# tiantengfei/Distributed-tensorflow-for-DCGAN

Hardware: AMD Instinct MI355X
Metric: images/sec (whole node), 64x64 DCGAN bs=128/GPU at 1/2/4/8 MI355X (higher is better)
Workload: dtype bf16; 1 GPU; model=DCGAN-64x64x3 (G 5,135,363 / D 4,316,545 params), global_batch=128, per_gpu_batch=128, parallelism=dp1, engine=hip, hip_graph=False, schedule=fused, backend=none, world_size=1

## Files before the change

### csrc/hip/narrow2.hip

```cpp
#include "kernels.h"

#if defined(DCG_F32)
extern "C" int DCG_API(dcg_nconv)(const elem_t*, const elem_t*, const float*, elem_t*, int, int, int, int, int, int,
                                  int, int, int, float, int, const elem_t*, const elem_t*, const float*, const float*,
                                  int, float, float*, hipStream_t) { return -2; }
extern "C" int DCG_API(dcg_nconv_tiles)(int, int, int) { return -1; }
extern "C" int DCG_API(dcg_nwgrad_plan)(int, int, int, int, int*, int*, int*) { return -1; }
extern "C" int DCG_API(dcg_nwgrad)(const elem_t*, int, int, int, int, const elem_t*, int, int, int, int, float*,
                                   hipStream_t) { return -2; }
extern "C" int DCG_API(dcg_narrow_deconv_dact)(const elem_t*, const elem_t*, elem_t*, const elem_t*, int, int, int, int,
                                               int, int, int, int, int, float, float*, hipStream_t) { return -2; }
extern "C" int DCG_API(dcg_narrow_deconv_tiles)(int, int, int) { return -1; }
extern "C" int DCG_API(dcg_wgrad3_taps_per_tile)(int) { return 1; }
extern "C" int DCG_API(dcg_narrow_deconv_bnin)(const elem_t*, const elem_t*, const float*, elem_t*, int, int, int, int,
                                               int, int, int, int, int, float, const float*, const float*, int, float,
                                               elem_t*, hipStream_t) { return -2; }
#else

namespace dcg {

constexpr int NC_TY = 4;
constexpr int NC_TX = 32;
constexpr int NC_WR = 2 * NC_TY + 3;
constexpr int NC_WC = 2 * NC_TX + 3;
constexpr int NC_WP = NC_WC + 1;
constexpr int NC_WPIX = NC_WR * NC_WC;
constexpr int NC_PPT = (NC_WPIX + 255) / 256;
constexpr int NC_KS = 136;
constexpr int NC_CS = 72;
constexpr int NC_SP = NC_TY * NC_TX * 8 / 256;

struct NConvArgs {
  const elem_t* x; const elem_t* w; const float* bias; elem_t* y;
  int H, W, Ho, Wo, pad_y, pad_x, act; float leak;
  int tiles_x, tiles_per_img, ntiles;
  const elem_t* bx; const elem_t* by; const float* mean; const float* rstd; int bact; float bleak;
  float* part;
};

template <int ACT>
__device__ __forceinline__ float nc_act(float v, float leak) {
  if constexpr (ACT == ACT_RELU) return fmaxf(v, 0.f);
  else if constexpr (ACT == ACT_LRELU) return fmaxf(v, leak * v);
  else if constexpr (ACT == ACT_TANH) return tanhf(v);
  else return v;
}

template <int CIN, bool BNB, int ACT>
__global__ __launch_bounds__(256) void nconv_kernel(NConvArgs p) {
  __shared__ __attribute__((aligned(16))) elem_t wt[64 * NC_KS];
  __shared__ __attribute__((aligned(16))) elem_t xs[NC_WR * NC_WP * 4];
  __shared__ float red[4][2][64];
  __shared__ __attribute__((aligned(16))) elem_t ct[NC_TY * NC_TX * NC_CS];
  const int tid = threadIdx.x, lane = tid & 63, wave = __builtin_amdgcn_readfirstlane(tid >> 6);
  const int li = lane & 15, g = lane >> 4;
  int t = blockIdx.x;
  if (t >= p.ntiles) return;

  for (int q = tid; q < 64 * NC_KS / 8; q += 256) reinterpret_cast<u32x4*>(wt)[q] = (u32x4){0u, 0u, 0u, 0u};
  __syncthreads();
  for (int q = tid; q < 25 * CIN * 64; q += 256) {
    const int n = q & 63, kk = q >> 6, tap = kk / CIN, c = kk - tap * CIN;
    wt[n * NC_KS + 4 * tap + c] = p.w[q];
  }
  __syncthreads();
  elem8 wf[4][4];
#pragma unroll
  for (int nb = 0; nb < 4; ++nb)
#pragma unroll
    for (int kb = 0; kb < 4; ++kb)
      wf[nb][kb] = *reinterpret_cast<const elem8*>(wt + (16 * nb + li) * NC_KS + 32 * kb + 8 * g);
  float bias_r[4][4];
#pragma unroll
  for (int nb = 0; nb < 4; ++nb)
#pragma unroll
    for (int e = 0; e < 4; ++e) bias_r[nb][e] = p.bias ? p.bias[16 * nb + 4 * g + e] : 0.f;
  const int c8 = tid & 7;
  float mu[8], rs[8], s1[8], s2[8];
#pragma unroll
  for (int e = 0; e < 8; ++e) {
    mu[e] = BNB ? p.mean[8 * c8 + e] : 0.f;
    rs[e] = BNB ? p.rstd[8 * c8 + e] : 0.f;
    s1[e] = 0.f;
    s2[e] = 0.f;
  }
  const float bslope = p.bact == ACT_LRELU ? p.bleak : 0.f;

  elem_t pv[NC_PPT][CIN];
  auto fetch = [&](int tt) {
    const int b = tt / p.tiles_per_img, rem = tt - b * p.tiles_per_img;
    const int ty = rem / p.tiles_x, tx = rem - ty * p.tiles_x;
    const int iy0 = 2 * ty * NC_TY - p.pad_y, ix0 = 2 * tx * NC_TX - p.pad_x;
#pragma unroll
    for (int i = 0; i < NC_PPT; ++i) {
      const int q = tid + 256 * i;
      const int r = q / NC_WC, c = q - r * NC_WC;
      const int iy = iy0 + r, ix = ix0 + c;
      const bool ok = q < NC_WPIX && (unsigned)iy < (unsigned)p.H && (unsigned)ix < (unsigned)p.W;
      const elem_t* src = p.x + (((size_t)b * p.H + (ok ? iy : 0)) * p.W + (ok ? ix : 0)) * CIN;
#pragma unroll
      for (int cc = 0; cc < CIN; ++cc) pv[i][cc] = ok ? src[cc] : (elem_t)0.f;
    }
  };
  auto commit = [&]() {
#pragma unroll
    for (int i = 0; i < NC_PPT; ++i) {
      const int q = tid + 256 * i;
      if (q < NC_WPIX) {
        const int r = q / NC_WC, c = q - r * NC_WC;
        elem4 v = {(elem_t)0.f, (elem_t)0.f, (elem_t)0.f, (elem_t)0.f};
#pragma unroll
        for (int cc = 0; cc < CIN; ++cc) v[cc] = pv[i][cc];
        *reinterpret_cast<elem4*>(xs + (r * NC_WP + c) * 4) = v;
      }
    }
  };
  fetch(t);
  commit();
  __syncthreads();
  for (; t < p.ntiles; t += gridDim.x) {
    const int tn = t + gridDim.x;
    const int b = t / p.tiles_per_img, rem = t - b * p.tiles_per_img;
    const int ty = rem / p.tiles_x, tx = rem - ty * p.tiles_x;
    f32x4 acc[2][4];
#pragma unroll
    for (int h = 0; h < 2; ++h)
#pragma unroll
      for (int nb = 0; nb < 4; ++nb) acc[h][nb] = (f32x4){0.f, 0.f, 0.f, 0.f};
#pragma unroll
    for (int kb = 0; kb < 4; ++kb) {
      const int t0 = min(8 * kb + 2 * g, 24), t1 = min(8 * kb + 2 * g + 1, 24);
      const int off0 = (t0 / 5) * NC_WP + (t0 % 5), off1 = (t1 / 5) * NC_WP + (t1 % 5);
#pragma unroll
      for (int h = 0; h < 2; ++h) {
        const int base = 2 * wave * NC_WP + 2 * (16 * h + li);
        const elem4 a0 = *reinterpret_cast<const elem4*>(xs + (base + off0) * 4);
        const elem4 a1 = *reinterpret_cast<const elem4*>(xs + (base + off1) * 4);
        const elem8 xf = __builtin_shufflevector(a0, a1, 0, 1, 2, 3, 4, 5, 6, 7);
#pragma unroll
        for (int nb = 0; nb < 4; ++nb) acc[h][nb] = DCG_MFMA_16x16x32(wf[nb][kb], xf, acc[h][nb], 0, 0, 0);
      }
    }
    if (tn < p.ntiles) fetch(tn);
#pragma unroll
    for (int h = 0; h < 2; ++h) {
      const int px = wave * NC_TX + 16 * h + li;
#pragma unroll
      for (int nb = 0; nb < 4; ++nb) {
        elem4 ov;
#pragma unroll
        for (int e = 0; e < 4; ++e) ov[e] = f2bf(nc_act<ACT>(acc[h][nb][e] + bias_r[nb][e], p.leak));
        *reinterpret_cast<elem4*>(ct + px * NC_CS + 16 * nb + 4 * g) = ov;
      }
    }
    __syncthreads();
    size_t o[NC_SP];
    bool ok[NC_SP];
#pragma unroll
    for (int i = 0; i < NC_SP; ++i) {
      const int px = (tid >> 3) + 32 * i;
      const int oy = ty * NC_TY + (px >> 5), ox = tx * NC_TX + (px & 31);
      ok[i] = oy < p.Ho && ox < p.Wo;
      o[i] = ok[i] ? (((size_t)b * p.Ho + oy) * p.Wo + ox) * 64 + 8 * c8 : 0;
    }
    elem8 bxv[NC_SP], byv[NC_SP];
    if constexpr (BNB) {
#pragma unroll
      for (int i = 0; i < NC_SP; ++i) {
        bxv[i] = *reinterpret_cast<const elem8*>(p.bx + o[i]);
        byv[i] = *reinterpret_cast<const elem8*>(p.by + o[i]);
      }
    }
#pragma unroll
    for (int i = 0; i < NC_SP; ++i) {
      const int px = (tid >> 3) + 32 * i;
      const u32x4 v = *reinterpret_cast<const u32x4*>(ct + px * NC_CS + 8 * c8);
      if (ok[i]) {
        *reinterpret_cast<u32x4*>(p.y + o[i]) = v;
        if constexpr (BNB) {
          const elem8 dv = __builtin_bit_cast(elem8, v);
#pragma unroll
          for (int e = 0; e < 8; ++e) {
            const float gv = (float)dv[e] * ((float)byv[i][e] > 0.f ? 1.f : bslope);
            s1[e] += gv;
            s2[e] += gv * ((float)bxv[i][e] - mu[e]) * rs[e];
          }
        }
      }
    }
    if (tn < p.ntiles) {
      commit();
      __syncthreads();
    }
  }
  if constexpr (BNB) {
#pragma unroll
    for (int e = 0; e < 8; ++e) {
      float a = s1[e], c = s2[e];
#pragma unroll
      for (int sh = 8; sh < 64; sh <<= 1) {
        a += __shfl_xor(a, sh, 64);
        c += __shfl_xor(c, sh, 64);
      }
      if (lane < 8) {
        red[wave][0][8 * c8 + e] = a;
        red[wave][1][8 * c8 + e] = c;
      }
    }
    __syncthreads();
    if (tid < 128) {
      const int st = tid >> 6, n = tid & 63;
      p.part[(size_t)blockIdx.x * 128 + tid] = ((red[0][st][n] + red[1][st][n]) + red[2][st][n]) + red[3][st][n];
    }
  }
}

constexpr int NWG_PX = 256;
constexpr int NWG_WIN = 2048;
constexpr int NWG_WPT = NWG_WIN / 256;

struct NWGradArgs {
  const elem_t* x; int H, W;
  const elem_t* d; int Hd, Wd;
  int pl;
  int tyc, np, nks;
  int wrows, wcols;
  int chunks_per_wg, wg_per_img;
  float* part;
};

__device__ __forceinline__ int nwg_swz(int r) {
  return 4 * (((r >> 1) & 1) | (((r >> 3) & 1) << 1));
}

template <int CIN>
__global__ __launch_bounds__(256) void nwgrad_kernel(NWGradArgs p) {
  extern __shared__ __attribute__((aligned(16))) char smem[];
  char* dt = smem;
  char* win = smem + NWG_PX * 128;
  const int tid = threadIdx.x, lane = tid & 63, wave = __builtin_amdgcn_readfirstlane(tid >> 6);
  const int li = lane & 15, g = lane >> 4, q = li >> 2, pp = li & 3;
  const int b = blockIdx.x / p.wg_per_img;
  const int yb = (blockIdx.x - b * p.wg_per_img) * p.chunks_per_wg * p.tyc;
  const int zero_pix = p.wrows * p.wcols;
  if (tid == 0) *reinterpret_cast<elem4*>(win + zero_pix * 8) = (elem4){(elem_t)0.f, (elem_t)0.f, (elem_t)0.f, (elem_t)0.f};

  int pxoff[8][2];
#pragma unroll
  for (int ks = 0; ks < 8; ++ks)
#pragma unroll
    for (int h = 0; h < 2; ++h) {
      const int px = min(32 * ks + 8 * g + 4 * h + q, p.np - 1);
      const int yy = px / p.Wd, xx = px - yy * p.Wd;
      pxoff[ks][h] = 2 * yy * p.wcols + 2 * xx;
    }
  const int mb0 = 2 * wave, nmb = wave < 3 ? 2 : 1;
  int tapoff[2];
  bool tapok[2];
#pragma unroll
  for (int i = 0; i < 2; ++i) {
    const int tap = 4 * (mb0 + i) + pp;
    tapok[i] = tap < 25;
    tapoff[i] = tapok[i] ? (tap / 5) * p.wcols + (tap % 5) : 0;
  }

  u32x4 dv[NWG_PX * 8 / 256];
  elem_t xv[NWG_WPT][CIN];
  int w_off[NWG_WPT], w_row[NWG_WPT];
#pragma unroll
  for (int i = 0; i < NWG_WPT; ++i) {
    const int s_ = tid + 256 * i;
    const int wr = s_ / p.wcols, wc = s_ - wr * p.wcols, ix = wc - p.pl;
    const bool col_ok = s_ < zero_pix && (unsigned)ix < (unsigned)p.W;
    w_row[i] = col_ok ? wr : -(1 << 20);
    w_off[i] = (wr * p.W + ix) * CIN;
  }
  auto fetch = [&](int y0) {
    const elem_t* dsrc = p.d + ((size_t)b * p.Hd + y0) * p.Wd * 64;
    const int lim = min(p.tyc, p.Hd - y0) * p.Wd * 64;
#pragma unroll
    for (int i = 0; i < NWG_PX * 8 / 256; ++i) {
      const int e0 = (tid + 256 * i) * 8;
      dv[i] = e0 < lim ? *reinterpret_cast<const u32x4*>(dsrc + e0) : (u32x4){0u, 0u, 0u, 0u};
    }
    const int iy0 = 2 * y0 - p.pl;
    const long long xbase = ((long long)b * p.H + iy0) * p.W * CIN;
#pragma unroll
    for (int i = 0; i < NWG_WPT; ++i) {
      const bool ok = (unsigned)(iy0 + w_row[i]) < (unsigned)p.H;
#pragma unroll
      for (int cc = 0; cc < CIN; ++cc) xv[i][cc] = ok ? p.x[xbase + w_off[i] + cc] : (elem_t)0.f;
    }
  };
  auto commit = [&]() {
#pragma unroll
    for (int i = 0; i < NWG_PX * 8 / 256; ++i) {
      const int qd = tid + 256 * i, px = qd >> 3, j = qd & 7;
      *reinterpret_cast<u32x4*>(dt + px * 128 + ((j ^ (nwg_swz(px) >> 1)) << 4)) = dv[i];
    }
#pragma unroll
    for (int i = 0; i < NWG_WPT; ++i) {
      const int s = tid + 256 * i;
      if (s < zero_pix) {
        elem4 v = {(elem_t)0.f, (elem_t)0.f, (elem_t)0.f, (elem_t)0.f};
#pragma unroll
        for (int cc = 0; cc < CIN; ++cc) v[cc] = xv[i][cc];
        *reinterpret_cast<elem4*>(win + s * 8) = v;
      }
    }
  };

  f32x4 acc[2][4];
#pragma unroll
  for (int i = 0; i < 2; ++i)
#pragma unroll
    for (int nb = 0; nb < 4; ++nb) acc[i][nb] = (f32x4){0.f, 0.f, 0.f, 0.f};

  const lds_char* dt3 = (const lds_char*)dt;
  const lds_char* win3 = (const lds_char*)win;
  int nch = 0;
  for (int c = 0; c < p.chunks_per_wg; ++c) nch += (yb + c * p.tyc < p.Hd) ? 1 : 0;
  if (nch > 0) {
    fetch(yb);
    commit();
  }
  __syncthreads();
  for (int c = 0; c < nch; ++c) {
    if (c + 1 < nch) fetch(yb + (c + 1) * p.tyc);
#pragma unroll
    for (int ks = 0; ks < 8; ++ks) {
      if (ks >= p.nks) break;
      elem8 bfr[4];
#pragma unroll
      for (int nb = 0; nb < 4; ++nb)
#pragma unroll
        for (int h = 0; h < 2; ++h) {
          const int r = 32 * ks + 8 * g + 4 * h + q;
          const s16x4 v = __builtin_amdgcn_ds_read_tr16_b64_v4i16(
              LDS_PTR(s16x4, dt3 + r * 128 + (((4 * nb + pp) ^ nwg_swz(r)) << 3)));
          const elem4 vb = __builtin_bit_cast(elem4, v);
#pragma unroll
          for (int e = 0; e < 4; ++e) bfr[nb][4 * h + e] = vb[e];
        }
#pragma unroll
      for (int i = 0; i < 2; ++i) {
        if (i < nmb) {
          elem8 af;
#pragma unroll
          for (int h = 0; h < 2; ++h) {
            const int pix = tapok[i] ? pxoff[ks][h] + tapoff[i] : zero_pix;
            const s16x4 v = __builtin_amdgcn_ds_read_tr16_b64_v4i16(LDS_PTR(s16x4, win3 + pix * 8));
            const elem4 va = __builtin_bit_cast(elem4, v);
#pragma unroll
            for (int e = 0; e < 4; ++e) af[4 * h + e] = va[e];
          }
#pragma unroll
          for (int nb = 0; nb < 4; ++nb) acc[i][nb] = DCG_MFMA_16x16x32(af, bfr[nb], acc[i][nb], 0, 0, 0);
        }
      }
    }
    __syncthreads();
    if (c + 1 < nch) {
      commit();
      __syncthreads();
    }
  }
  float* dst = p.part + (size_t)blockIdx.x * 25 * CIN * 64;
#pragma unroll
  for (int i = 0; i < 2; ++i) {
    if (i < nmb) {
      const int tap = 4 * (mb0 + i) + g;
      if (tap < 25) {
#pragma unroll
        for (int nb = 0; nb < 4; ++nb)
#pragma unroll
          for (int e = 0; e < CIN; ++e) dst[(tap * CIN + e) * 64 + 16 * nb + li] = acc[i][nb][e];
      }
    }
  }
}

}

using namespace dcg;

extern "C" int DCG_API(dcg_nconv)(const elem_t* x, const elem_t* w, const float* bias, elem_t* y, int B, int H, int W,
                                  int Cin, int Ho, int Wo, int pad_y, int pad_x, int act, float leak, int grid,
                                  const elem_t* bx, const elem_t* by, const float* mean, const float* rstd, int bact,
                                  float bleak, float* part, hipStream_t s) {
  if (Cin < 1 || Cin > 4 || pad_y < 0 || pad_y > 2 || pad_x < 0 || pad_x > 2) return -2;
  if (Ho != (H + 1) / 2 || Wo != (W + 1) / 2) return -2;
  NConvArgs a{};
  a.x = x; a.w = w; a.bias = bias; a.y = y;
  a.H = H; a.W = W; a.Ho = Ho; a.Wo = Wo; a.pad_y = pad_y; a.pad_x = pad_x; a.act = act; a.leak = leak;
  a.tiles_x = (Wo + NC_TX - 1) / NC_TX;
  a.tiles_per_img = a.tiles_x * ((Ho + NC_TY - 1) / NC_TY);
  a.ntiles = B * a.tiles_per_img;
  if (grid < 1 || grid > a.ntiles) return -2;
  a.bx = bx; a.by = by; a.mean = mean; a.rstd = rstd; a.bact = bact; a.bleak = bleak; a.part = part;
  const bool bnb = bx != nullptr;
  if (bnb && (!by || !mean || !rstd || !part)) return -2;
#define NC_ACT(CI, BB)                                                                              \
  switch (act) {                                                                                    \
    case ACT_RELU: hipLaunchKernelGGL((nconv_kernel<CI, BB, ACT_RELU>), dim3(grid), dim3(256), 0, s, a); break;   \
    case ACT_LRELU: hipLaunchKernelGGL((nconv_kernel<CI, BB, ACT_LRELU>), dim3(grid), dim3(256), 0, s, a); break; \
    case ACT_TANH: hipLaunchKernelGGL((nconv_kernel<CI, BB, ACT_TANH>), dim3(grid), dim3(256), 0, s, a); break;   \
    default: hipLaunchKernelGGL((nconv_kernel<CI, BB, ACT_NONE>), dim3(grid), dim3(256), 0, s, a); break;         \
  }
#define NC_LAUNCH(CI)    \
  if (bnb) {             \
    NC_ACT(CI, true)     \
  } else {               \
    NC_ACT(CI, false)    \
  }
  switch (Cin) {
    case 1: NC_LAUNCH(1) break;
    case 2: NC_LAUNCH(2) break;
    case 3: NC_LAUNCH(3) break;
    default: NC_LAUNCH(4) break;
  }
#undef NC_LAUNCH
#undef NC_ACT
  return (int)hipGetLastError();
}

extern "C" int DCG_API(dcg_nconv_tiles)(int B, int Ho, int Wo) {
  return B * ((Wo + NC_TX - 1) / NC_TX) * ((Ho + NC_TY - 1) / NC_TY);
}

extern "C" int DCG_API(dcg_nwgrad_plan)(int H, int W, int Hd, int Wd, int* tyc, int* wrows, int* wcols) {
  if (Wd < 1 || Wd > NWG_PX || Hd < 1 || W > 2 * Wd + 1 || H > 2 * Hd + 1) return -1;
  const int t = NWG_PX / Wd;
  const int wr = 2 * t + 3, wc = 2 * Wd + 3;
  if (wr * wc > NWG_WIN) return -1;
  *tyc = t; *wrows = wr; *wcols = wc;
  return 0;
}

extern "C" int DCG_API(dcg_nwgrad)(const elem_t* x, int B, int H, int W, int Cin, const elem_t* d, int Hd, int Wd,
                                   int pl, int chunks_per_wg, float* part, hipStream_t s) {
  NWGradArgs a{};
  if (Cin < 1 || Cin > 4 || pl < 0 || pl > 2 || chunks_per_wg < 1) return -2;
  if (DCG_API(dcg_nwgrad_plan)(H, W, Hd, Wd, &a.tyc, &a.wrows, &a.wcols)) return -2;
  a.x = x; a.H = H; a.W = W; a.d = d; a.Hd = Hd; a.Wd = Wd; a.pl = pl;
  a.np = a.tyc * Wd;
  a.nks = (a.np + 31) / 32;
  a.chunks_per_wg = chunks_per_wg;
  const int chunks_per_img = (Hd + a.tyc - 1) / a.tyc;
  a.wg_per_img = (chunks_per_img + chunks_per_wg - 1) / chunks_per_wg;
  a.part = part;
  const size_t shm = (size_t)NWG_PX * 128 + (size_t)(a.wrows * a.wcols + 1) * 8;
  const unsigned grid = (unsigned)(B * a.wg_per_img);
#define NW_LAUNCH(CI)                                                                                       \
  {                                                                                                         \
    static bool attr = false;                                                                               \
    if (!attr) {                                                                                            \
      hipError_t e = hipFuncSetAttribute((const void*)nwgrad_kernel<CI>, hipFuncAttributeMaxDynamicSharedMemorySize, \
                                         (int)(NWG_PX * 128 + (NWG_WIN + 1) * 8));                          \
      if (e != hipSuccess) return (int)e;                                                                   \
      attr = true;                                                                                          \
    }                                                                                                       \
    hipLaunchKernelGGL(nwgrad_kernel<CI>, dim3(grid), dim3(256), shm, s, a);                                \
  }
  switch (Cin) {
    case 1: NW_LAUNCH(1) break;
    case 2: NW_LAUNCH(2) break;
    case 3: NW_LAUNCH(3) break;
    default: NW_LAUNCH(4) break;
  }
#undef NW_LAUNCH
  return (int)hipGetLastError();
}
#endif
```

Before: 133,100 images/sec.

## Restructure narrow conv staging: vector row loads, LDS aliasing, prefetched BN operands

```diff
diff --git a/csrc/hip/narrow2.hip b/csrc/hip/narrow2.hip
--- a/csrc/hip/narrow2.hip
+++ b/csrc/hip/narrow2.hip
@@ -36,7 +36,11 @@
   int tiles_x, tiles_per_img, ntiles;
   const elem_t* bx; const elem_t* by; const float* mean; const float* rstd; int bact; float bleak;
   float* part;
+  unsigned x_bytes;
+  unsigned y_img_bytes;
 };
+
+typedef unsigned int nc_u32x4 __attribute__((ext_vector_type(4), aligned(2)));
 
 template <int ACT>
 __device__ __forceinline__ float nc_act(float v, float leak) {
@@ -46,82 +50,145 @@
   else return v;
 }
 
-template <int CIN, bool BNB, int ACT>
-__global__ __launch_bounds__(256) void nconv_kernel(NConvArgs p) {
-  __shared__ __attribute__((aligned(16))) elem_t wt[64 * NC_KS];
+template <int CIN, bool BNB, int ACT, bool FAST>
+__global__ __launch_bounds__(256, 2) void nconv_kernel(NConvArgs p) {
+  __shared__ __attribute__((aligned(16))) elem_t ct[NC_TY * NC_TX * NC_CS];
   __shared__ __attribute__((aligned(16))) elem_t xs[NC_WR * NC_WP * 4];
   __shared__ float red[4][2][64];
-  __shared__ __attribute__((aligned(16))) elem_t ct[NC_TY * NC_TX * NC_CS];
+  __shared__ __attribute__((aligned(16))) float cst[4][64];
+  static_assert(64 * NC_KS <= NC_TY * NC_TX * NC_CS, "the weight matrix is staged in the C tile's LDS");
+  elem_t* const wt = ct;
   const int tid = threadIdx.x, lane = tid & 63, wave = __builtin_amdgcn_readfirstlane(tid >> 6);
   const int li = lane & 15, g = lane >> 4;
   int t = blockIdx.x;
   if (t >= p.ntiles) return;
-
-  for (int q = tid; q < 64 * NC_KS / 8; q += 256) reinterpret_cast<u32x4*>(wt)[q] = (u32x4){0u, 0u, 0u, 0u};
-  __syncthreads();
-  for (int q = tid; q < 25 * CIN * 64; q += 256) {
-    const int n = q & 63, kk = q >> 6, tap = kk / CIN, c = kk - tap * CIN;
-    wt[n * NC_KS + 4 * tap + c] = p.w[q];
-  }
-  __syncthreads();
-  elem8 wf[4][4];
-#pragma unroll
-  for (int nb = 0; nb < 4; ++nb)
-#pragma unroll
-    for (int kb = 0; kb < 4; ++kb)
-      wf[nb][kb] = *reinterpret_cast<const elem8*>(wt + (16 * nb + li) * NC_KS + 32 * kb + 8 * g);
-  float bias_r[4][4];
-#pragma unroll
-  for (int nb = 0; nb < 4; ++nb)
-#pragma unroll
-    for (int e = 0; e < 4; ++e) bias_r[nb][e] = p.bias ? p.bias[16 * nb + 4 * g + e] : 0.f;
   const int c8 = tid & 7;
-  float mu[8], rs[8], s1[8], s2[8];
-#pragma unroll
-  for (int e = 0; e < 8; ++e) {
-    mu[e] = BNB ? p.mean[8 * c8 + e] : 0.f;
-    rs[e] = BNB ? p.rstd[8 * c8 + e] : 0.f;
-    s1[e] = 0.f;
-    s2[e] = 0.f;
-  }
-  const float bslope = p.bact == ACT_LRELU ? p.bleak : 0.f;
-
-  elem_t pv[NC_PPT][CIN];
+
+  auto out_of = [&](int tt, size_t& img, int& o0, int& nv) {
+    const int b = tt / p.tiles_per_img, rem = tt - b * p.tiles_per_img;
+    const int ty = rem / p.tiles_x, tx = rem - ty * p.tiles_x;
+    const int ox = tx * NC_TX + (tid >> 3), oy0 = ty * NC_TY;
+    nv = ox < p.Wo ? min(NC_TY, p.Ho - oy0) : 0;
+    o0 = (oy0 * p.Wo + ox) * 64 + 8 * c8;
+    img = (size_t)b * p.Ho * p.Wo * 64;
+  };
+  const int orow = p.Wo * 64;
+  auto load_bn = [&](size_t img, int o0, int nv, elem8 (&vx)[NC_SP], elem8 (&vy)[NC_SP]) {
+#pragma unroll
+    for (int i = 0; i < NC_SP; ++i) {
+      const size_t o = i < nv ? img + (o0 + i * orow) : 0;
+      vx[i] = *reinterpret_cast<const elem8*>(p.bx + o);
+      vy[i] = *reinterpret_cast<const elem8*>(p.by + o);
+    }
+  };
+
+  elem_t pv[FAST ? 1 : NC_PPT][CIN];
+  u32x4 pw[FAST ? CIN : 1];
+  const int f_g = p.W >> 3, f_r = tid / max(f_g, 1), f_j = tid - f_r * f_g;
+  const bool f_on = f_r < NC_WR;
+  const __amdgpu_buffer_rsrc_t rx = make_rsrc(p.x, FAST ? p.x_bytes : 0u);
   auto fetch = [&](int tt) {
     const int b = tt / p.tiles_per_img, rem = tt - b * p.tiles_per_img;
     const int ty = rem / p.tiles_x, tx = rem - ty * p.tiles_x;
     const int iy0 = 2 * ty * NC_TY - p.pad_y, ix0 = 2 * tx * NC_TX - p.pad_x;
-#pragma unroll
-    for (int i = 0; i < NC_PPT; ++i) {
-      const int q = tid + 256 * i;
-      const int r = q / NC_WC, c = q - r * NC_WC;
-      const int iy = iy0 + r, ix = ix0 + c;
-      const bool ok = q < NC_WPIX && (unsigned)iy < (unsigned)p.H && (unsigned)ix < (unsigned)p.W;
-      const elem_t* src = p.x + (((size_t)b * p.H + (ok ? iy : 0)) * p.W + (ok ? ix : 0)) * CIN;
-#pragma unroll
-      for (int cc = 0; cc < CIN; ++cc) pv[i][cc] = ok ? src[cc] : (elem_t)0.f;
+    if constexpr (FAST) {
+      const int iy = iy0 + f_r;
+      const bool ok = f_on && (unsigned)iy < (unsigned)p.H;
+      const uint32_t off = (uint32_t)(((b * p.H + iy) * p.W + 8 * f_j) * CIN) * 2u;
+#pragma unroll
+      for (int cc = 0; cc < CIN; ++cc) pw[cc] = buf_load16(rx, oob_unless(ok, off + 16u * cc));
+    } else {
+#pragma unroll
+      for (int i = 0; i < NC_PPT; ++i) {
+        const int q = tid + 256 * i;
+        const int r = q / NC_WC, c = q - r * NC_WC;
+        const int iy = iy0 + r, ix = ix0 + c;
+        const bool ok = q < NC_WPIX && (unsigned)iy < (unsigned)p.H && (unsigned)ix < (unsigned)p.W;
+        const elem_t* src = p.x + (((size_t)b * p.H + (ok ? iy : 0)) * p.W + (ok ? ix : 0)) * CIN;
+#pragma unroll
+        for (int cc = 0; cc < CIN; ++cc) pv[i][cc] = ok ? src[cc] : (elem_t)0.f;
+      }
     }
   };
   auto commit = [&]() {
-#pragma unroll
-    for (int i = 0; i < NC_PPT; ++i) {
-      const int q = tid + 256 * i;
-      if (q < NC_WPIX) {
-        const int r = q / NC_WC, c = q - r * NC_WC;
-        elem4 v = {(elem_t)0.f, (elem_t)0.f, (elem_t)0.f, (elem_t)0.f};
-#pragma unroll
-        for (int cc = 0; cc < CIN; ++cc) v[cc] = pv[i][cc];
-        *reinterpret_cast<elem4*>(xs + (r * NC_WP + c) * 4) = v;
+    if constexpr (FAST) {
+      if (f_on) {
+        elem_t ev[8 * CIN];
+#pragma unroll
+        for (int cc = 0; cc < CIN; ++cc) {
+          const elem8 v = __builtin_bit_cast(elem8, pw[cc]);
+#pragma unroll
+          for (int k = 0; k < 8; ++k) ev[8 * cc + k] = v[k];
+        }
+#pragma unroll
+        for (int j = 0; j < 8; ++j) {
+          elem4 v = {(elem_t)0.f, (elem_t)0.f, (elem_t)0.f, (elem_t)0.f};
+#pragma unroll
+          for (int cc = 0; cc < CIN; ++cc) v[cc] = ev[j * CIN + cc];
+          *reinterpret_cast<elem4*>(xs + (f_r * NC_WP + p.pad_x + 8 * f_j + j) * 4) = v;
+        }
+      }
+    } else {
+#pragma unroll
+      for (int i = 0; i < NC_PPT; ++i) {
+        const int q = tid + 256 * i;
+        if (q < NC_WPIX) {
+          const int r = q / NC_WC, c = q - r * NC_WC;
+          elem4 v = {(elem_t)0.f, (elem_t)0.f, (elem_t)0.f, (elem_t)0.f};
+#pragma unroll
+          for (int cc = 0; cc < CIN; ++cc) v[cc] = pv[i][cc];
+          *reinterpret_cast<elem4*>(xs + (r * NC_WP + c) * 4) = v;
+        }
       }
     }
   };
+
+  size_t img;
+  int o0, nv;
+  out_of(t, img, o0, nv);
   fetch(t);
+  elem8 bxv[NC_SP], byv[NC_SP];
+  if constexpr (BNB) load_bn(img, o0, nv, bxv, byv);
+  const int wtap = tid >> 3, wn = tid & 7;
+  u32x4 wv[CIN];
+#pragma unroll
+  for (int cc = 0; cc < CIN; ++cc) {
+    const int row = min(wtap * CIN + cc, 25 * CIN - 1);
+    wv[cc] = *reinterpret_cast<const nc_u32x4*>(p.w + row * 64 + 8 * wn);
+  }
+  const float* cp = tid < 64 ? p.bias : !BNB ? nullptr : tid < 128 ? p.mean : tid < 192 ? p.rstd : nullptr;
+  const float cv = cp ? cp[tid & 63] : 0.f;
+  if constexpr (FAST) {
+    for (int q = tid; q < NC_WR * NC_WP * 4 / 8; q += 256) reinterpret_cast<u32x4*>(xs)[q] = (u32x4){0u, 0u, 0u, 0u};
+    __syncthreads();
+  }
+  cst[tid >> 6][tid & 63] = cv;
+#pragma unroll
+  for (int j = 0; j < 8; ++j) {
+    elem4 v = {(elem_t)0.f, (elem_t)0.f, (elem_t)0.f, (elem_t)0.f};
+#pragma unroll
+    for (int cc = 0; cc < CIN; ++cc) v[cc] = wtap < 25 ? __builtin_bit_cast(elem8, wv[cc])[j] : (elem_t)0.f;
+    *reinterpret_cast<elem4*>(wt + (8 * wn + j) * NC_KS + 4 * wtap) = v;
+  }
+  __syncthreads();
+  elem8 wf[4][4];
+#pragma unroll
+  for (int nb = 0; nb < 4; ++nb)
+#pragma unroll
+    for (int kb = 0; kb < 4; ++kb)
+      wf[nb][kb] = *reinterpret_cast<const elem8*>(wt + (16 * nb + li) * NC_KS + 32 * kb + 8 * g);
+  float s1[8], s2[8];
+#pragma unroll
+  for (int e = 0; e < 8; ++e) {
+    s1[e] = 0.f;
+    s2[e] = 0.f;
+  }
+  const float bslope = p.bact == ACT_LRELU ? p.bleak : 0.f;
   commit();
   __syncthreads();
-  for (; t < p.ntiles; t += gridDim.x) {
+  for (;;) {
     const int tn = t + gridDim.x;
-    const int b = t / p.tiles_per_img, rem = t - b * p.tiles_per_img;
-    const int ty = rem / p.tiles_x, tx = rem - ty * p.tiles_x;
+    const bool more = tn < p.ntiles;
     f32x4 acc[2][4];
 #pragma unroll
     for (int h = 0; h < 2; ++h)
@@ -141,42 +208,47 @@
         for (int nb = 0; nb < 4; ++nb) acc[h][nb] = DCG_MFMA_16x16x32(wf[nb][kb], xf, acc[h][nb], 0, 0, 0);
       }
     }
-    if (tn < p.ntiles) fetch(tn);
+    size_t imgn = 0;
+    int o0n = 0, nvn = 0;
+    elem8 bxn[NC_SP], byn[NC_SP];
+    if (more) {
+      out_of(tn, imgn, o0n, nvn);
+      fetch(tn);
+      if constexpr (BNB) load_bn(imgn, o0n, nvn, bxn, byn);
+    }
 #pragma unroll
     for (int h = 0; h < 2; ++h) {
       const int px = wave * NC_TX + 16 * h + li;
 #pragma unroll
       for (int nb = 0; nb < 4; ++nb) {
+        const f32x4 bs = *reinterpret_cast<const f32x4*>(&cst[0][16 * nb + 4 * g]);
         elem4 ov;
 #pragma unroll
-        for (int e = 0; e < 4; ++e) ov[e] = f2bf(nc_act<ACT>(acc[h][nb][e] + bias_r[nb][e], p.leak));
+        for (int e = 0; e < 4; ++e) ov[e] = f2bf(nc_act<ACT>(acc[h][nb][e] + bs[e], p.leak));
         *reinterpret_cast<elem4*>(ct + px * NC_CS + 16 * nb + 4 * g) = ov;
       }
     }
     __syncthreads();
-    size_t o[NC_SP];
-    bool ok[NC_SP];
-#pragma unroll
-    for (int i = 0; i < NC_SP; ++i) {
-      const int px = (tid >> 3) + 32 * i;
-      const int oy = ty * NC_TY + (px >> 5), ox = tx * NC_TX + (px & 31);
-      ok[i] = oy < p.Ho && ox < p.Wo;
-      o[i] = ok[i] ? (((size_t)b * p.Ho + oy) * p.Wo + ox) * 64 + 8 * c8 : 0;
-    }
-    elem8 bxv[NC_SP], byv[NC_SP];
+    const __amdgpu_buffer_rsrc_t ry = make_rsrc(p.y + img, p.y_img_bytes);
+    float mu[8], rs[8];
     if constexpr (BNB) {
 #pragma unroll
-      for (int i = 0; i < NC_SP; ++i) {
-        bxv[i] = *reinterpret_cast<const elem8*>(p.bx + o[i]);
-        byv[i] = *reinterpret_cast<const elem8*>(p.by + o[i]);
+      for (int h = 0; h < 2; ++h) {
+        const f32x4 m4 = *reinterpret_cast<const f32x4*>(&cst[1][8 * c8 + 4 * h]);
+        const f32x4 r4 = *reinterpret_cast<const f32x4*>(&cst[2][8 * c8 + 4 * h]);
+#pragma unroll
+        for (int e = 0; e < 4; ++e) {
+          mu[4 * h + e] = m4[e];
+          rs[4 * h + e] = r4[e];
+        }
       }
     }
 #pragma unroll
     for (int i = 0; i < NC_SP; ++i) {
       const int px = (tid >> 3) + 32 * i;
       const u32x4 v = *reinterpret_cast<const u32x4*>(ct + px * NC_CS + 8 * c8);
-      if (ok[i]) {
-        *reinterpret_cast<u32x4*>(p.y + o[i]) = v;
+      __builtin_amdgcn_raw_buffer_store_b128(v, ry, oob_unless(i < nv, (uint32_t)(o0 + i * orow) * 2u), 0, 0);
+      if (i < nv) {
         if constexpr (BNB) {
           const elem8 dv = __builtin_bit_cast(elem8, v);
 #pragma unroll
@@ -188,9 +260,19 @@
         }
       }
     }
-    if (tn < p.ntiles) {
-      commit();
-      __syncthreads();
+    if (!more) break;
+    commit();
+    __syncthreads();
+    t = tn;
+    img = imgn;
+    o0 = o0n;
+    nv = nvn;
+    if constexpr (BNB) {
+#pragma unroll
+      for (int i = 0; i < NC_SP; ++i) {
+        bxv[i] = bxn[i];
+        byv[i] = byn[i];
+      }
     }
   }
   if constexpr (BNB) {
@@ -400,18 +482,28 @@
   a.bx = bx; a.by = by; a.mean = mean; a.rstd = rstd; a.bact = bact; a.bleak = bleak; a.part = part;
   const bool bnb = bx != nullptr;
   if (bnb && (!by || !mean || !rstd || !part)) return -2;
-#define NC_ACT(CI, BB)                                                                              \
+  const size_t x_bytes = (size_t)B * H * W * Cin * sizeof(elem_t);
+  const bool fast = a.tiles_x == 1 && W % 8 == 0 && ((uintptr_t)x & 15) == 0 && x_bytes < OOB;
+  a.x_bytes = fast ? (unsigned)x_bytes : 0u;
+  const size_t y_img_bytes = (size_t)Ho * Wo * 64 * sizeof(elem_t);
+  if (y_img_bytes >= OOB) return -2;
+  a.y_img_bytes = (unsigned)y_img_bytes;
+#define NC_ACT(CI, BB, FF)                                                                          \
   switch (act) {                                                                                    \
-    case ACT_RELU: hipLaunchKernelGGL((nconv_kernel<CI, BB, ACT_RELU>), dim3(grid), dim3(256), 0, s, a); break;   \
-    case ACT_LRELU: hipLaunchKernelGGL((nconv_kernel<CI, BB, ACT_LRELU>), dim3(grid), dim3(256), 0, s, a); break; \
-    case ACT_TANH: hipLaunchKernelGGL((nconv_kernel<CI, BB, ACT_TANH>), dim3(grid), dim3(256), 0, s, a); break;   \
-    default: hipLaunchKernelGGL((nconv_kernel<CI, BB, ACT_NONE>), dim3(grid), dim3(256), 0, s, a); break;         \
-  }
-#define NC_LAUNCH(CI)    \
-  if (bnb) {             \
-    NC_ACT(CI, true)     \
-  } else {               \
-    NC_ACT(CI, false)    \
+    case ACT_RELU: hipLaunchKernelGGL((nconv_kernel<CI, BB, ACT_RELU, FF>), dim3(grid), dim3(256), 0, s, a); break;   \
+    case ACT_LRELU: hipLaunchKernelGGL((nconv_kernel<CI, BB, ACT_LRELU, FF>), dim3(grid), dim3(256), 0, s, a); break; \
+    case ACT_TANH: hipLaunchKernelGGL((nconv_kernel<CI, BB, ACT_TANH, FF>), dim3(grid), dim3(256), 0, s, a); break;   \
+    default: hipLaunchKernelGGL((nconv_kernel<CI, BB, ACT_NONE, FF>), dim3(grid), dim3(256), 0, s, a); break;         \
+  }
+#define NC_LAUNCH(CI)          \
+  if (bnb && fast) {           \
+    NC_ACT(CI, true, true)     \
+  } else if (bnb) {            \
+    NC_ACT(CI, true, false)    \
+  } else if (fast) {           \
+    NC_ACT(CI, false, true)    \
+  } else {                     \
+    NC_ACT(CI, false, false)   \
   }
   switch (Cin) {
     case 1: NC_LAUNCH(1) break;
```

Result: no change. 134,400 images/sec (median of 6 runs) (+1.0%).
